# schreibfaul1/ESP32-Opus-Player

Measured on AMD Instinct MI355X. Metric: decoded 48 kHz stereo frames/sec/GPU (x real-time); HBM GB/s vs roofline, higher is better.
Workload: dtype int32 fixed-point (int16/int32 with 64-bit products); 1 GPU; celt_fb_stereo_64k; streams_per_gpu=65536

## Files before the change

__graft_entry__.py:

```python
import importlib.util
import os
import subprocess
import sys

ROOT = os.path.dirname(os.path.abspath(__file__))
PKG_DIR = os.path.join(ROOT, "esp32-opus-player_amd")
CSRC = os.path.join(PKG_DIR, "csrc")


def _load_pkg():
    name = "esp32_opus_player_amd"
    if name in sys.modules:
        return sys.modules[name]
    path = os.path.join(PKG_DIR, "__init__.py")
    spec = importlib.util.spec_from_file_location(name, path, submodule_search_locations=[PKG_DIR])
    mod = importlib.util.module_from_spec(spec)
    sys.modules[name] = mod
    spec.loader.exec_module(mod)
    return mod


def build() -> None:
    subprocess.check_call([sys.executable, os.path.join(ROOT, "tools", "gen_rom_tables.py")])
    hipcc = os.environ.get("HIPCC", "/opt/rocm/bin/hipcc")
    out = os.path.join(PKG_DIR, "libopusgpu.so")
    cmd = [hipcc, "--offload-arch=gfx950", "-O3", "-std=c++17", "-fPIC", "-shared",
           os.path.join(CSRC, "og_api.hip"), os.path.join(CSRC, "og_recon.hip"), os.path.join(CSRC, "og_parse64.hip"), os.path.join(CSRC, "og_rfc.hip"), os.path.join(CSRC, "og_silk_nb.hip"), os.path.join(CSRC, "og_silk_synth.hip"), os.path.join(CSRC, "og_compat.cpp"),
           os.path.join(CSRC, "og_pages.cpp"), os.path.join(CSRC, "og_files.cpp"),
           "-I", os.path.join(ROOT, "include"), "-pthread",
           "-o", out]
    cmd = [c for c in cmd if not c.endswith("og_compat.cpp") or os.path.exists(c)]
    flags_file = os.path.join(CSRC, "BUILD_FLAGS")
    if os.path.exists(flags_file):
        cmd += open(flags_file).read().split()
    subprocess.check_call(cmd)
    subprocess.check_call(["make", "-C", os.path.join(ROOT, "oracle"), "-s"])
    emul = os.path.join(ROOT, "tests", "emul")
    if os.path.exists(os.path.join(emul, "Makefile")):
        subprocess.check_call(["make", "-C", emul, "-s"])
    kat = os.path.join(ROOT, "tests", "gpu_kat")
    if os.path.exists(os.path.join(kat, "Makefile")):
        subprocess.check_call(["make", "-C", kat, "-s", "HIPCC=" + hipcc])
    pkg = _load_pkg()
    lib = pkg.load_lib()
    missing = [s for s in pkg.EXPORTS if not hasattr(lib, s)]
    if missing:
        raise RuntimeError(f"libopusgpu.so lacks exports: {missing}")


def smoke() -> None:
    import numpy as np
    sys.path.insert(0, os.path.join(ROOT, "tests"))
    import oracle_py
    pkg = _load_pkg()
    oracle = oracle_py.load()
    ctx = pkg.Context(0)
    n, frames = 64, 3
    for name, toc, L in (("CELT-FB", pkg.TOC_CELT_FB_STEREO, 160), ("SILK-NB", pkg.TOC_SILK_NB_STEREO, 40),
                         ("hybrid FB", pkg.TOC_HYBRID_FB_STEREO, 120)):
        pay = pkg.lcg_payloads(n, frames, L)
        ref, ok = oracle.batch_decode(2, toc, pay)
        assert ok == n * frames
        ctx.streams_alloc(n, 2)
        for f in range(frames):
            pk = [bytes([toc]) + pay[f, s].tobytes() for s in range(n)]
            pcm, res = ctx.decode_packets(np.arange(n), pk)
            assert (res == 960).all(), (name, res)
            assert (pcm == ref[:, f]).all(), f"{name}: GPU PCM differs from the oracle"
    ctx.close()
    print("smoke ok: 64 streams x 3 frames x {CELT-FB, SILK-NB, hybrid FB} bit-exact vs oracle")


if __name__ == "__main__":
    build()
    if len(sys.argv) > 1 and sys.argv[1] == "smoke":
        smoke()
```

esp32-opus-player_amd/csrc/og_api.hip:

```cpp
#include <hip/hip_runtime.h>
#include <stdio.h>
#include <stdlib.h>
#include <string.h>
#include <condition_variable>
#include <functional>
#include <memory>
#include <new>
#include <mutex>
#include <thread>
#include <vector>
#include "og_decode.hpp"
#include "og_host_framing.hpp"
#include "og_output.hpp"
#include "og_debug.hpp"

using namespace og;

static_assert(sizeof(opusgpu_frame_desc) == sizeof(FrameDesc), "descriptor layout");

#define OG_STALL_MAX_SPINS (1 << 20)
__global__ void __launch_bounds__(64) k_stream_stall(long long ticks, int max_spins) {
    const long long t0 = wall_clock64();
    for (int i = 0; i < max_spins && wall_clock64() - t0 < ticks; i++) __builtin_amdgcn_s_sleep(8);
}
// ... 212 lines not shown
            ret = BAD_ARG;
        } else if (desc_rfc(d.flags)) {
            continue;
        } else if (skip_celt && desc_mode(d.flags) == MODE_CELT) {
            continue;
        } else {
            StreamState *s = &st[d.stream];
#ifdef OG_PROF_SINGLE
            OG_PROF_INIT();
#endif
            ret = decode_frame_wave<true>(s, arena + d.offset, d.len, desc_mode(d.flags), desc_bandwidth(d.flags),
                                          desc_channels(d.flags), pcm + (size_t)f * pcm_stride, handoff ? &handoff[f] : nullptr,
                                          srecs ? &srecs[f] : nullptr, q4_only, desc_mode_after(d.flags));
#ifdef OG_PROF_SINGLE
            OG_PROF_FLUSH();
#endif
            if (ret == CONTINUE_SPLIT) continue;
        }
        if (threadIdx.x == 0) result[f] = ret;
        __syncthreads();
    }
}

extern "C" void og_launch_silk_synth(hipStream_t s, const void *descs, const void *arena, void *streams, void *pcm, void *result, int n,
                                     int n_streams, int pcm_stride, void *handoff, const void *srecs, int nb_elsewhere);
extern "C" void og_launch_silk_synth_nb(hipStream_t s, const void *descs, const void *arena, void *streams, void *pcm, void *result, int n,
                                        int n_streams, int pcm_stride, void *handoff, const void *srecs, int nb_elsewhere);

#define OG_SPARSE_WAVES 4
template <int LANES>
OG_DEV void silk_parse_kernel_body(const FrameDesc *__restrict__ descs, const u8 *__restrict__ arena, const StreamState *st, SilkRec *srecs,
                                   SilkHandoff *handoff, int n, int n_streams, SilkShadow *shadow, u32 epoch) {
    silk_tables_load();
    if ((int)threadIdx.x >= LANES) return;
    const int f = (int)blockIdx.x * LANES + (int)threadIdx.x;
    if (f >= n) return;
    const FrameDesc d = descs[f];
    const int mode = desc_mode(d.flags);
    if (d.stream < 0 || d.stream >= n_streams || mode == MODE_CELT || desc_rfc(d.flags)) return;
#ifdef OG_PROF_SPARSE
    OG_PROF_INIT();
#endif
    SilkShadow *const sh = shadow ? &shadow[d.stream] : nullptr;
    const SilkPast past(&st[d.stream], sh, epoch);
    silk_parse_lane(past, arena + d.offset, d.len, mode, desc_bandwidth(d.flags), desc_channels(d.flags), &srecs[f], &handoff[f], sh, epoch,
                    desc_mode_after(d.flags));
#ifdef OG_PROF_SPARSE
    OG_PROF_FLUSH();
#endif
}
__global__ void __launch_bounds__(64, OG_SPARSE_WAVES) k_silk_parse(const FrameDesc *__restrict__ descs, const u8 *__restrict__ arena,
                                                      const StreamState *st, SilkRec *srecs, SilkHandoff *handoff, int n,
                                                      int n_streams, SilkShadow *shadow, u32 epoch) {
    silk_parse_kernel_body<32>(descs, arena, st, srecs, handoff, n, n_streams, shadow, epoch);
}
__global__ void __launch_bounds__(64, OG_SPARSE_WAVES) k_silk_parse64(const FrameDesc *__restrict__ descs, const u8 *__restrict__ arena,
                                                        const StreamState *st, SilkRec *srecs, SilkHandoff *handoff, int n,
                                                        int n_streams, SilkShadow *shadow, u32 epoch) {
    silk_parse_kernel_body<64>(descs, arena, st, srecs, handoff, n, n_streams, shadow, epoch);
}

#define OG_SPARAMS_WAVES 4
__global__ void __launch_bounds__(64, OG_SPARAMS_WAVES) k_silk_params(const FrameDesc *__restrict__ descs, const StreamState *st, SilkRec *srecs,
                                                                       int n, int n_streams, SilkShadow *shadow, u32 epoch) {
    constexpr int FR = OG_PAR_LANES / 2;
    const int ch = (int)threadIdx.x / FR, f = (int)blockIdx.x * FR + (int)threadIdx.x % FR;
    bool act = f < n;
    FrameDesc d = {0, 0, 0, 0};
    if (act) {
        d = descs[f];
        act = !(d.stream < 0 || d.stream >= n_streams || desc_mode(d.flags) == MODE_CELT || desc_rfc(d.flags));
    }
    SilkShadow *const sh = act && shadow ? &shadow[d.stream] : nullptr;
    const SilkParPast past(act ? &st[d.stream] : st, sh, epoch);
    const int mode = desc_mode(d.flags), channels = desc_channels(d.flags);
    SilkParTask t;
    t.skip = 1;
    if (act) silk_params_channel(past, mode, desc_bandwidth(d.flags), channels, &srecs[f], ch, t);
    OG_FULL_SYNC();
    if (act) silk_params_shadow(past, t, channels, &srecs[f], ch, sh, epoch);
}

#define OG_PARSE_KERNEL_NAME k_celt_parse
#include "og_parse_kernel.hpp"
extern "C" void og_launch_celt_parse64(hipStream_t s, int grid, const void *descs, const void *arena, void *streams, void *recs, int n,
                                       int n_streams, const void *handoff, int which, int groups, unsigned *started);
extern "C" int og_celt_parse64_frames(void);

extern "C" void og_launch_celt_recon_fb(hipStream_t s, const void *descs, void *streams, const void *recs, void *rout, int n,
                                        int n_streams, int hybrid, unsigned *started, int empties);
extern "C" int og_celt_recon_fb_signals(int n);
extern "C" void og_launch_decode_rfc(hipStream_t s, const void *descs, const void *arena, void *streams, void *pcm, void *result, int n,
                                     int n_streams, int pcm_stride);
__global__ void __launch_bounds__(64, OG_RECON_WAVES) k_celt_recon(const FrameDesc *__restrict__ descs, StreamState *st,
                                                                      const ParseRec *recs, ReconOut *rout, int n,
                                                                      int n_streams, int hybrid, int rest_only) {
    unsigned long long todo = 1ull;
    int base = (int)blockIdx.x;
    if (rest_only) {
        base = (int)blockIdx.x * 64;
        const int f0 = base + (int)threadIdx.x;
        bool mine = false;
        if (f0 < n) {
            const FrameDesc d0 = descs[f0];
            const int m0 = desc_mode(d0.flags);
            if (d0.stream >= 0 && d0.stream < n_streams && (m0 == MODE_CELT || (m0 == MODE_HYBRID && hybrid)) && !desc_rfc(d0.flags)) {
                const u32 fl = recs[f0].flags;
                const bool fast = !(fl & (RF_SKIP | RF_BAD_CELT)) && ((fl >> RF_LM_SHIFT) & 3) == 3 && recs[f0].n_words < REC_MAX_WORDS &&
                                  recs[f0].n_leaves <= FAST_MAX_LEAVES;
                mine = !fast && !(m0 == MODE_HYBRID && (fl & RF_SKIP));
            }
        }
        todo = __ballot(mine);
    }
    while (todo) {
        const int f = base + (int)__builtin_ctzll(todo);
        todo &= todo - 1;
        if (f >= n) return;
        const FrameDesc d = descs[f];
        const int mode = desc_mode(d.flags);
        if (d.stream < 0 || d.stream >= n_streams || !(mode == MODE_CELT || (mode == MODE_HYBRID && hybrid)) || desc_rfc(d.flags)) continue;
        if (mode == MODE_HYBRID && (recs[f].flags & RF_SKIP)) continue;
#if !defined(OG_PROF_PARSE) && !defined(OG_PROF_SINGLE) && !defined(OG_PROF_SPARSE) && !defined(OG_PROF_SSYNTH)
        OG_PROF_INIT();
#endif
        const int pos = OG_UNI(st[d.stream].celt.ring_pos);
        const int ret = celt_recon_wave(&st[d.stream], &recs[f], mode, desc_channels(d.flags), rest_only ? RECON_REST_ONLY : RECON_ALL, desc_mode_after(d.flags));
        if (ret != RECON_NOT_MINE && threadIdx.x == 0) rout[f] = ReconOut{ret, pos};
#if !defined(OG_PROF_PARSE) && !defined(OG_PROF_SINGLE) && !defined(OG_PROF_SPARSE) && !defined(OG_PROF_SSYNTH)
        OG_PROF_FLUSH();
#endif
        __syncthreads();
    }
}

static __device__ __forceinline__ i32 pk_add_sat_i16(i32 a, i32 b) {
    typedef short s2 __attribute__((ext_vector_type(2)));
    const s2 r = __builtin_elementwise_add_sat(__builtin_bit_cast(s2, a), __builtin_bit_cast(s2, b));
    return __builtin_bit_cast(i32, r);
}
template <class T>
static __device__ __forceinline__ T *uniform_ptr(T *p) {
    const unsigned long long a = (unsigned long long)p;
    return (T *)((unsigned long long)(u32)__builtin_amdgcn_readfirstlane((int)(u32)a) |
                 (unsigned long long)(u32)__builtin_amdgcn_readfirstlane((int)(u32)(a >> 32)) << 32);
}
#define OG_POST_WAVES 5
__global__ void __launch_bounds__(64, OG_POST_WAVES) k_celt_post(const FrameDesc *__restrict__ descs, StreamState *st, const ParseRec *recs,
                                                  const ReconOut *__restrict__ rout, i32 *__restrict__ result, i16 *pcm, int n,
                                                  int n_streams, int channels, int pcm_stride, const SilkHandoff *handoff,
                                                  int modes, int others_ran) {
    constexpr int CS = 32, PCS = CS / 4, RSTEP = 64 / PCS;
    static_assert(RSTEP % 2 == 0, "a lane's rows are all of one channel");
    __shared__ __attribute__((aligned(16))) i32 tin[64][CS + 4];
    const int lane = (int)threadIdx.x;
    const int t = (int)blockIdx.x * 64 + lane;
    const int f = channels == 2 ? t >> 1 : t, c = channels == 2 ? t & 1 : 0;
    bool live = false, emit = false;
    StreamState *ss = nullptr;
    const i16 *silk = nullptr;
    int silk_n = 0;
    int pos = 0, stream = 0;
    if (f < n) {
        const FrameDesc d = descs[f];
        stream = d.stream;
        const int mode = desc_mode(d.flags);
        const bool stream_ok = d.stream >= 0 && d.stream < n_streams;
// ... 157 lines not shown
    const int per = (wide ? og_celt_parse64_frames() : OG_PL_FRAMES) * ctx->parse_groups;
    return (cnt + per - 1) / per;
}
void launch_celt_parse(opusgpu_ctx *ctx, hipStream_t q, const Step &st, size_t f0, int cnt, bool wide, bool early) {
    const StepRange r(st, f0);
    const int which = early ? (int)PARSE_CELT_ONLY : (int)PARSE_ALL, groups = early ? ctx->parse_groups : 1;
    const int per = wide ? og_celt_parse64_frames() : OG_PL_FRAMES;
    const int grid = early ? celt_parse_early_grid(ctx, cnt, wide) : (cnt + per - 1) / per;
    u32 *const started = early ? ctx->sp.d_started : nullptr;
    if (wide)
        og_launch_celt_parse64(q, grid, r.dd, st.arena, ctx->d_streams, r.recs, cnt, ctx->n_streams, r.hh, which, groups, started);
    else
        hipLaunchKernelGGL(k_celt_parse, dim3(grid), dim3(64 * OG_PL_WAVES), 0, q, r.dd, (const u8 *)st.arena, ctx->d_streams, r.recs, cnt,
                           ctx->n_streams, (const SilkHandoff *)r.hh, which, groups, started);
}
void launch_celt_recon_fb(opusgpu_ctx *ctx, hipStream_t q, const Step &st, size_t f0, int cnt, bool counts_in) {
    const StepRange r(st, f0);
    ctx->recon_fb_took_rest = counts_in && !r.hh && st.modes == 4 && og_debug().rest_in_fb;
    og_launch_celt_recon_fb(q, r.dd, ctx->d_streams, r.recs, r.rout, cnt, ctx->n_streams, r.hh ? 1 : 0, counts_in ? ctx->sp.d_started + 16 : nullptr,
                            ctx->recon_fb_took_rest ? 1 : 0);
}
void launch_celt_recon(opusgpu_ctx *ctx, hipStream_t q, const Step &st, size_t f0, int cnt) {
    if (ctx->fast_recon && ctx->recon_fb_took_rest) {
        ctx->recon_fb_took_rest = false;
        return;
    }
    const StepRange r(st, f0);
    hipLaunchKernelGGL(k_celt_recon, dim3(ctx->fast_recon ? (cnt + 63) / 64 : cnt), dim3(64), 0, q, r.dd, ctx->d_streams, (const ParseRec *)r.recs,
                       r.rout, cnt, ctx->n_streams, r.hh ? 1 : 0, ctx->fast_recon);
}
void launch_celt_post(opusgpu_ctx *ctx, hipStream_t q, const Step &st, size_t f0, int cnt, bool others) {
    const StepRange r(st, f0);
    hipLaunchKernelGGL(k_celt_post, dim3((cnt * ctx->channels + 63) / 64), dim3(64), 0, q, r.dd, ctx->d_streams, (const ParseRec *)r.recs,
                       (const ReconOut *)r.rout, r.rr, r.pp, cnt, ctx->n_streams, ctx->channels, st.pcm_stride, (const SilkHandoff *)r.hh, st.modes,
                       others ? 1 : 0);
}
void launch_silk_synth(opusgpu_ctx *ctx, hipStream_t q, const Step &st, size_t f0, int cnt, int nb_done) {
    const StepRange r(st, f0);
    og_launch_silk_synth(q, r.dd, st.arena, ctx->d_streams, r.pp, r.rr, cnt, ctx->n_streams, st.pcm_stride, r.hh, r.srecs, nb_done);
}
void launch_silk_synth_nb(opusgpu_ctx *ctx, hipStream_t q, const Step &st, size_t f0, int cnt) {
    const StepRange r(st, f0);
    og_launch_silk_synth_nb(q, r.dd, st.arena, ctx->d_streams, r.pp, r.rr, cnt, ctx->n_streams, st.pcm_stride, r.hh, r.srecs, 1);
}


extern "C" {


int opusgpu_version(void) { return 100; }

int opusgpu_ctx_create(int device, opusgpu_ctx **out) {
    if (!out || device < 0) return OPUSGPU_BAD_ARG;
    *out = nullptr;
    int count = 0;
    if (hipGetDeviceCount(&count) != hipSuccess || count <= 0 || device >= count) return OPUSGPU_ERR_NO_DEVICE;
    if (hipSetDevice(device) != hipSuccess) return OPUSGPU_ERR_NO_DEVICE;
    hipFuncAttributes attr;
    if (hipFuncGetAttributes(&attr, reinterpret_cast<const void *>(k_decode_step)) != hipSuccess) {
        (void)hipGetLastError();
        return OPUSGPU_ERR_NO_DEVICE;
    }
    opusgpu_ctx *ctx = new (std::nothrow) opusgpu_ctx();
    if (!ctx) return OPUSGPU_ALLOC_FAIL;
    ctx->device = device;
    ctx->split_celt = og_debug().split;
    ctx->split_hybrid = og_debug().split_hybrid;
    ctx->fast_recon = og_debug().fast_recon;
    ctx->parse_groups = og_debug().parse_groups;
    ctx->host_parts = og_debug().host_parts;
    if (og_debug().stall_us) {
        int khz = 0;
        if (hipDeviceGetAttribute(&khz, hipDeviceAttributeWallClockRate, device) != hipSuccess || khz <= 0) {
            (void)hipGetLastError();
            delete ctx;
            return OPUSGPU_ERR_HIP;
        }
        ctx->stall_ticks = (long long)og_debug().stall_us * khz / 1000;
    }
    if (hipStreamCreateWithFlags(&ctx->stream, hipStreamNonBlocking) != hipSuccess) {
        delete ctx;
        return OPUSGPU_ERR_HIP;
    }
    *out = ctx;
    return OPUSGPU_OK;
}

void opusgpu_ctx_destroy(opusgpu_ctx *ctx) {
    if (!ctx) return;
    (void)hipSetDevice(ctx->device);
    (void)hipStreamSynchronize(ctx->stream);
    (void)hipFree(ctx->d_streams);
    (void)hipFree(ctx->d_descs);
    (void)hipFree(ctx->d_arena);
    (void)hipFree(ctx->d_pcm);
    (void)hipFree(ctx->d_result);
    pipeline_destroy(ctx);
    for (int i = 0; i < 6; i++) {
        (void)hipFree(ctx->d_recs[i]);
        (void)hipFree(ctx->d_rout[i]);
    }
    for (int i = 0; i < OG_SILK_SETS; i++) {
        (void)hipFree(ctx->d_handoff[i]);
        (void)hipFree(ctx->d_srecs[i]);
    }
    (void)hipFree(ctx->d_shadow);
    (void)hipHostFree(ctx->h_pcm);
    (void)hipHostFree(ctx->h_res);
    (void)hipHostFree(ctx->h_arena);
    (void)hipHostFree(ctx->h_descs);
    (void)hipFree(ctx->d_crc_tables);
    for (hipEvent_t e : ctx->ev_piece)
        if (e) (void)hipEventDestroy(e);
    for (hipEvent_t e : ctx->ev_part)
        if (e) (void)hipEventDestroy(e);
    if (ctx->copy_stream) (void)hipStreamDestroy(ctx->copy_stream);
    (void)hipStreamDestroy(ctx->stream);
    delete ctx;
}

const char *opusgpu_last_error(const opusgpu_ctx *ctx) { return ctx ? ctx->err : "no context"; }
int opusgpu_set_mode(opusgpu_ctx *ctx, int mode) {
    if (!ctx || (mode != OPUSGPU_MODE_REFERENCE && mode != OPUSGPU_MODE_RFC)) return OPUSGPU_BAD_ARG;
    ctx->mode = mode;
    return OPUSGPU_OK;
}
int opusgpu_get_mode(const opusgpu_ctx *ctx) { return ctx ? ctx->mode : OPUSGPU_MODE_REFERENCE; }
int opusgpu_set_pipeline(opusgpu_ctx *ctx, int on) {
    if (!ctx) return OPUSGPU_BAD_ARG;
    HIPCHK(ctx, hipSetDevice(ctx->device));
    if (on)
        if (int rc = pipeline_create(ctx)) return rc;
    if ((on != 0) != (ctx->pipeline != 0)) {
        HIPCHK(ctx, hipDeviceSynchronize());
        ctx->sp.drained();
        ctx->sp.last_kind = 0;
        ctx->sp.shadow_epoch++;
    }
    ctx->pipeline = on ? 1 : 0;
    return OPUSGPU_OK;
}
int opusgpu_get_pipeline(const opusgpu_ctx *ctx) { return ctx ? ctx->pipeline : 0; }
size_t opusgpu_stream_state_bytes(void) { return sizeof(StreamState); }
int opusgpu_stream_count(const opusgpu_ctx *ctx) { return ctx ? ctx->n_streams : 0; }
int opusgpu_stream_channels(const opusgpu_ctx *ctx) { return ctx ? ctx->channels : 0; }

int opusgpu_streams_reset(opusgpu_ctx *ctx, int first, int count, int full) {
    if (!ctx || first < 0 || count < 0 || first + count > ctx->n_streams) return OPUSGPU_BAD_ARG;
    if (count == 0) return OPUSGPU_OK;
    HIPCHK(ctx, hipSetDevice(ctx->device));
    if (int rc = sync_in_flight(ctx)) return rc;
    ctx->sp.drained();
    ctx->sp.shadow_epoch++;
    hipLaunchKernelGGL(k_stream_init, dim3(count), dim3(64), 0, ctx->stream, ctx->d_streams, first, count, ctx->channels,
                       full ? 1 : 0);
    HIPCHK(ctx, hipGetLastError());
    HIPCHK(ctx, hipStreamSynchronize(ctx->stream));
    for (int i = first; i < first + count; i++) ctx->last_count[i] = ctx->last_flags[i] = 0;
    return OPUSGPU_OK;
}

int opusgpu_streams_alloc(opusgpu_ctx *ctx, int n_streams, int channels) {
    if (!ctx || n_streams <= 0 || (channels != 1 && channels != 2)) return OPUSGPU_BAD_ARG;
    HIPCHK(ctx, hipSetDevice(ctx->device));
    HIPCHK(ctx, hipStreamSynchronize(ctx->stream));
    if (int rc = sync_in_flight(ctx)) return rc;
// ... 385 lines not shown
```

esp32-opus-player_amd/csrc/og_celt_parse.hpp:

```cpp
#pragma once
#include "og_celt.hpp"
#include "og_celt_rec.hpp"

namespace og {

#ifndef OG_PL_LANES
#define OG_PL_LANES (OG_NLANES >= 32 ? 32 : OG_NLANES)
#endif
#ifndef OG_PL_WAVES
#define OG_PL_WAVES 1
#endif
#ifdef OG_HOST_EMUL
#define OG_PWAVE 0
#define OG_PCOL OG_LANE
#else
#define OG_PWAVE ((int)(threadIdx.x >> 6))
#define OG_PCOL ((int)(threadIdx.x & 63))
#endif
#define OG_PL_FRAMES (OG_PL_LANES * OG_PL_WAVES)
struct ParseLds {
    i8 fine_quant[NBANDS][OG_PL_LANES];
    i8 tf_prio[NBANDS][OG_PL_LANES];
    union {
        i16 bandE[2 * NBANDS][OG_PL_LANES];
        struct {
            u32 bw[NBANDS][OG_PL_LANES];
        } al;
        i32 stack[4][5][OG_PL_LANES];
    } u;
};
#ifdef OG_PARSE_DYN_LDS
extern __shared__ __attribute__((aligned(16))) unsigned char og_dyn_lds[];
#define PLs (reinterpret_cast<ParseLds *>(og_dyn_lds))
#else
OG_LDS ParseLds PLs[OG_PL_WAVES];
#endif
#define PL PLs[OG_PWAVE]

struct ParseTabLds {
    i16 eband[NBANDS + 1], logn[NBANDS];
    u16 pulse_idx[105];
    u32 pulse_v[392];
    u8 pulse_bits[392], band_alloc[231], pulse_caps[168], log2_frac[24], eprob[336];
};
#ifdef OG_PARSE_DYN_LDS
#define PT (*reinterpret_cast<ParseTabLds *>(og_dyn_lds + sizeof(ParseLds) * OG_PL_WAVES))
#define OG_PARSE_LDS_BYTES (sizeof(ParseLds) * OG_PL_WAVES + sizeof(ParseTabLds))
#else
OG_LDS ParseTabLds PT;
#define OG_PARSE_LDS_BYTES 0
#endif
struct RomLds {
    static OG_MEMBER i32 eband(int i) { return PT.eband[i]; }
    static OG_MEMBER i32 logn(int i) { return PT.logn[i]; }
    static OG_MEMBER i32 pulse_idx(int i) { return PT.pulse_idx[i]; }
    static OG_MEMBER i32 pulse_bits(int i) { return PT.pulse_bits[i]; }
    static OG_MEMBER i32 band_alloc(int i) { return PT.band_alloc[i]; }
    static OG_MEMBER i32 pulse_caps(int i) { return PT.pulse_caps[i]; }
    static OG_MEMBER i32 log2_frac(int i) { return PT.log2_frac[i]; }
    static OG_MEMBER i32 eprob(int i) { return PT.eprob[i]; }
};
OG_DEV void parse_tables_load() {
    OG_FOR_LANES(i, NBANDS + 1) PT.eband[i] = rom_eband[i];
    OG_FOR_LANES(i, NBANDS) PT.logn[i] = rom_logn[i];
    OG_FOR_LANES(i, 105) PT.pulse_idx[i] = rom_pulse_idx[i];
    OG_FOR_LANES(i, 392) PT.pulse_bits[i] = rom_pulse_bits[i];
    OG_FOR_LANES(i, 392) PT.pulse_v[i] = rom_pulse_v[i];
    OG_FOR_LANES(i, 231) PT.band_alloc[i] = rom_band_alloc[i];
    OG_FOR_LANES(i, 168) PT.pulse_caps[i] = rom_pulse_caps[i];
    OG_FOR_LANES(i, 24) PT.log2_frac[i] = rom_log2_frac[i];
    OG_FOR_LANES(i, 336) PT.eprob[i] = rom_eprob[i];
    OG_FULL_SYNC();
}

struct TfResView {
    i8 *p;
    OG_MEMBER operator int() const { return (int)(i8)((u8)*p << 4) >> 4; }
    OG_MEMBER void operator=(int v) const { *p = (i8)((*p & 0xF0) | (v & 15)); }
};
struct FinePrioView {
    i8 *p;
    OG_MEMBER operator int() const { return (*p >> 4) & 1; }
    OG_MEMBER void operator=(int v) const { *p = (i8)((*p & ~0x10) | ((v & 1) << 4)); }
};
struct LaneArr {
// ... 10 lines not shown
        for (int i = 0; i < NBANDS; i++) w[i] = *reinterpret_cast<const u32 *>(&rest[2 * i]);
        for (int i = 0; i < NBANDS; i++) {
            PL.u.bandE[2 * i][OG_PCOL] = (i16)(w[i] & 0xffff);
            PL.u.bandE[2 * i + 1][OG_PCOL] = (i16)(w[i] >> 16);
        }
    }
    typedef u16 __attribute__((may_alias)) u16a;
    typedef i32 __attribute__((may_alias)) i32a;
    OG_MEMBER i32 &pulses(int i) const { return pl[i]; }
    OG_MEMBER i32a &alloc_bits(int i) const { return *reinterpret_cast<i32a *>(&PL.u.al.bw[i][OG_PCOL]); }
    OG_MEMBER void pulses_rest(int start, int end) const {
        i32 v[24];
        for (int i = 0; i < 24; i++) v[i] = (i >= start && i < end) ? (i32)PL.u.al.bw[i < NBANDS ? i : 0][OG_PCOL] : 0;
#ifdef OG_HOST_EMUL
        for (int i = 0; i < NBANDS; i++) pl[i] = v[i];
#else
        typedef i32 i32x4 __attribute__((ext_vector_type(4)));
        for (int i = 0; i < 24; i += 4) *reinterpret_cast<i32x4 *>(&pl[i]) = i32x4{v[i], v[i + 1], v[i + 2], v[i + 3]};
#endif
        for (int i = 0; i < NBANDS; i++) pk[i] = (i16)v[i];
    }
    OG_MEMBER i8 &fine_quant(int i) const { return PL.fine_quant[i][OG_PCOL]; }
    OG_MEMBER FinePrioView fine_prio(int i) const { return FinePrioView{&PL.tf_prio[i][OG_PCOL]}; }
    OG_MEMBER TfResView tf_res(int i) const { return TfResView{&PL.tf_prio[i][OG_PCOL]}; }
    OG_MEMBER void boost_put(int i, int n, int) const {
#ifdef OG_HOST_EMUL
        if (n < 0 || n > 127) __builtin_trap();
#endif
        PL.fine_quant[i][OG_PCOL] = (i8)n;
    }
    OG_MEMBER i32 boost(int i, int C, int LM) const { return (i32)PL.fine_quant[i][OG_PCOL] * dynalloc_quanta<RomLds>(i, LM, C); }
    OG_MEMBER u16a &bits1(int i) const { return reinterpret_cast<u16a *>(&PL.u.al.bw[i][OG_PCOL])[0]; }
    OG_MEMBER u16a &bits2(int i) const { return reinterpret_cast<u16a *>(&PL.u.al.bw[i][OG_PCOL])[1]; }
    OG_MEMBER i16 &bandE(int i) const { return PL.u.bandE[i][OG_PCOL]; }
};

struct RecWriter {
    ParseRec *rec;
    int nw, nl, ncoef = 0;
    int job = 0;
    OG_MEMBER void word(u32 w) {
        if (nw < REC_MAX_WORDS) rec->words[nw] = w;
        nw++;
    }
    OG_MEMBER int reserve() { return nw++; }
    OG_MEMBER void patch(int at, u32 w) {
        if (at < REC_MAX_WORDS) rec->words[at] = w;
    }
    OG_MEMBER void leaf(int x, int N, int K, int B, i32 gain, int off, u32 idx) {
        if (nl < REC_MAX_LEAVES) {
            const u32 geom = (u32)x | (u32)N << 11 | (u32)K << 19 | (u32)(B - 1) << 27;
            const u32 aux = (u32)(gain & 0xffff) | (u32)off << 16 | (u32)job << 20;
#ifdef OG_HOST_EMUL
            rec->leaf[nl].idx = idx; rec->leaf[nl].geom = geom; rec->leaf[nl].aux = aux; rec->leaf[nl].pad = 0;
#else
            typedef u32 u32x4 __attribute__((ext_vector_type(4)));
            *reinterpret_cast<u32x4 *>(&rec->leaf[nl]) = u32x4{idx, geom, aux, 0u};
#endif
        }
        nl++;
        ncoef += N;
    }
    OG_MEMBER int band_begin() { return nw = (nw + 3) & ~3; }
    OG_MEMBER void words4(u32 w0, u32 w1, u32 w2, u32 w3) {
        if (nw + 4 <= REC_MAX_WORDS) {
#ifdef OG_HOST_EMUL
            rec->words[nw] = w0; rec->words[nw + 1] = w1; rec->words[nw + 2] = w2; rec->words[nw + 3] = w3;
#else
            typedef u32 u32x4 __attribute__((ext_vector_type(4)));
            *reinterpret_cast<u32x4 *>(&rec->words[nw]) = u32x4{w0, w1, w2, w3};
#endif
        }
        nw += 4;
    }
};

OG_DEV u32 isqrt24(u32 val) {
    u32 g = (u32)__builtin_sqrtf((float)val);
    g -= g * g > val;
    g += (g + 1) * (g + 1) <= val;
    return g;
}

OG_DEV void split_theta_lane(RcLane &rc, int band, Split &sc, int N, i32 &b, int B0, int LM) {
    int itheta = 0;
    const int pulse_cap = RomLds::logn(band) + LM * (1 << BITRES);
    const int offset = (pulse_cap >> 1) - 4;
    const int qn = compute_qn(N, b, offset, pulse_cap, 0);
    const u32 tell = rc_tell_frac(rc);
    if (qn != 1) {
        const bool uni = B0 > 1;
        const int h = qn >> 1;
        const int ftb = uni ? OG_MAX(ilog((u32)qn) - 8, 0) : 0;
        const u32 ft = uni ? (u32)(qn >> ftb) + 1 : (u32)((h + 1) * (h + 1));
        const u32 fm = rc_decode(rc, ft);
        const bool low = fm < (u32)(h * (h + 1) >> 1);
        const u32 root = isqrt24(8 * (low ? fm : ft - fm - 1) + 1);
        const int it = low ? (int)((root - 1) >> 1) : (int)((2u * (u32)(qn + 1) - root) >> 1);
        const int fs_t = low ? it + 1 : qn + 1 - it;
        const u32 fl_t = low ? (u32)(it * (it + 1) >> 1) : ft - (u32)(fs_t * (fs_t + 1) >> 1);
        const u32 fl = uni ? fm : fl_t, fs = uni ? 1u : (u32)fs_t;
        rc_update(rc, fl, fl + fs, ft);
        itheta = uni ? (int)fm : it;
        if (ftb) {
            const u32 t = fm << ftb | rc_bits(rc, (unsigned)ftb);
            if (t > (u32)qn) rc.error = 1;
            itheta = (int)OG_MIN(t, (u32)qn);
        }
        itheta = (int)udiv((u32)(itheta * 16384), (u32)qn);
    }
    const int qalloc = (int)(rc_tell_frac(rc) - tell);
    b -= qalloc;
    int imid, iside, delta;
    if (itheta == 0) {
        imid = 32767;
        iside = 0;
        delta = -16384;
    } else if (itheta == 16384) {
        imid = 0;
        iside = 32767;
        delta = 16384;
    } else {
        imid = bitexact_cos(itheta);
        iside = bitexact_cos(16384 - itheta);
        delta = frac_mul16((N - 1) << 7, bitexact_log2tan(iside, imid));
    }
    sc.inv = 0;
    sc.imid = imid;
    sc.iside = iside;
    sc.delta = delta;
    sc.itheta = itheta;
    sc.qalloc = qalloc;
}

OG_DEV int parse_tree(RcLane &rc, RecWriter &out, int band, i32 &remaining_bits, int x, int N, i32 b, int B, int LM, i32 gain,
                      int has_low, int silent) {
    int depth = 0, off = 0, n_fill = 0;
    const int jpos = out.reserve(), first_pvq = out.nl;
    for (;;) {
        OG_MARK(41);
        for (;;) {
            if (!(LM != -1 && b > pulse_cache_max<RomLds>(band, LM) + 12 && N > 2)) break;
            const int B0 = B;
            Split sc;
            N >>= 1;
            LM -= 1;
            B = (B + 1) >> 1;
            split_theta_lane(rc, band, sc, N, b, B0, LM);
            i32 delta = sc.delta;
            const int itheta = sc.itheta;
            if (B0 > 1 && (itheta & 0x3fff)) {
                if (itheta > 8192)
                    delta -= delta >> (4 - LM);
                else
                    delta = OG_MIN(0, delta + (N << BITRES >> (5 - LM)));
            }
            const i32 mbits = OG_MAX(0, OG_MIN(b, (b - delta) / 2));
            const i32 sbits = b - mbits;
            remaining_bits -= sc.qalloc;
            const int mid_first = mbits >= sbits;
            const int off_side = off + (B0 >> 1), silent_mid = silent | (itheta == 16384), silent_side = silent | (itheta == 0);
            const i32 gain_mid = tr16(mul16_p15(gain, sc.imid)), gain_side = tr16(mul16_p15(gain, sc.iside));
#ifdef OG_HOST_EMUL
            if (x + N >= 2048 || N > 255 || LM + 1 > 7 || B > 31 || off_side > 15) __builtin_trap();
#endif
            i32 *F = &PL.u.stack[depth][0][OG_PCOL];
            F[0 * OG_PL_LANES] = (i32)((u32)(mid_first ? x + N : x) | (u32)N << 11 | (u32)(LM + 1) << 19 | (u32)B << 22 |
                                       (u32)(mid_first ? off_side : off) << 27 | (u32)(mid_first ? silent_side : silent_mid) << 31);
            F[1 * OG_PL_LANES] = mid_first ? mbits : sbits;
            F[2 * OG_PL_LANES] = mid_first ? sbits : mbits;
            F[3 * OG_PL_LANES] = remaining_bits;
            F[4 * OG_PL_LANES] = ((mid_first ? gain_side : gain_mid) & 0xffff) | (itheta != (mid_first ? 0 : 16384)) << 16;
            depth++;
            if (mid_first) {
                b = mbits;
                gain = gain_mid;
                silent = silent_mid;
            } else {
                x += N;
                b = sbits;
                gain = gain_side;
                off = off_side;
                silent = silent_side;
            }
        }
        {
            OG_MARK(42);
            int q = bits2pulses<RomLds>(band, LM, b), curr_bits = pulses2bits<RomLds>(band, LM, q);
            remaining_bits -= curr_bits;
            while (remaining_bits < 0 && q > 0) {
                remaining_bits += curr_bits;
                q--;
                curr_bits = pulses2bits<RomLds>(band, LM, q);
                remaining_bits -= curr_bits;
            }
            const int K = q ? get_pulses(q) : 0;
            OG_MARK(43);
            if (K)
                out.leaf(x, N, K, B, gain, off, rc_uint(rc, PT.pulse_v[pulse_cache<RomLds>(band, LM) + q]));
            else if (!silent) {
                out.word((u32)off << LW_OFF_SHIFT | (u32)(B - 1) << LW_B_SHIFT | (u32)N << LW_N_SHIFT);
                out.word((u32)x | (u32)(gain & 0xffff) << 11);
                n_fill++;
            }
        }
        OG_MARK(44);
        if (depth == 0) break;
        {
            depth--;
// ... 256 lines not shown
```

esp32-opus-player_amd/csrc/og_parse64.hip:

```cpp
#include <hip/hip_runtime.h>
#define OG_PL_LANES 64
#define OG_PL_WAVES 2
#define OG_PARSE_KERNEL_NAME k_celt_parse64
#define OG_PARSE_DYN_LDS 1
#define OG_PARSE_WAVES_PER_SIMD 3
#ifndef OG_PARSE_NUM_VGPR
#define OG_PARSE_NUM_VGPR 152
#endif
#include "og_parse_kernel.hpp"

extern "C" void og_launch_celt_parse64(hipStream_t s, int grid, const void *descs, const void *arena, void *streams, void *recs, int n,
                                       int n_streams, const void *handoff, int which, int groups, unsigned *started) {
    hipLaunchKernelGGL(k_celt_parse64, dim3(grid), dim3(64 * OG_PL_WAVES), OG_PARSE_LDS_BYTES, s, (const FrameDesc *)descs, (const u8 *)arena, (StreamState *)streams,
                       (ParseRec *)recs, n, n_streams, (const SilkHandoff *)handoff, which, groups, started);
}
extern "C" int og_celt_parse64_frames(void) { return OG_PL_FRAMES; }

static_assert(sizeof(ParseLds) == (size_t)OG_PL_LANES * (2 * NBANDS + 4 * NBANDS), "a parse wave's LDS: fine_quant, tf_prio and one word per band");
static_assert(sizeof(ParseLds) <= 8064 && OG_PARSE_LDS_BYTES + 256 <= 16 * 1280, "k_celt_parse64's workgroup no longer fits 16 LDS granules");
static_assert((128 - 2 * ((OG_PARSE_LDS_BYTES + 256 + 1279) / 1280)) / 5 >= 19, "fewer than 19 reconstruction workgroups per CU beside two parse workgroups");
extern "C" int og_celt_parse64_lds_bytes(void) { return (int)OG_PARSE_LDS_BYTES; }
```

esp32-opus-player_amd/csrc/og_parse_kernel.hpp:

```cpp
#pragma once
#include "og_celt_parse.hpp"

using namespace og;

enum { PARSE_ALL = 0, PARSE_CELT_ONLY = 1, PARSE_HYBRID_ONLY = 2 };
#ifndef OG_PARSE_WAVES_PER_SIMD
#define OG_PARSE_WAVES_PER_SIMD 2
#endif
#ifdef OG_PARSE_NUM_VGPR
#define OG_PARSE_VGPR_ATTR __attribute__((amdgpu_num_vgpr(OG_PARSE_NUM_VGPR / 2)))
#else
#define OG_PARSE_VGPR_ATTR
#endif
__global__ void OG_PARSE_VGPR_ATTR __attribute__((amdgpu_waves_per_eu(OG_PARSE_WAVES_PER_SIMD, 8))) __launch_bounds__(64 * OG_PL_WAVES) OG_PARSE_KERNEL_NAME(const FrameDesc *__restrict__ descs, const u8 *__restrict__ arena,
                                                      StreamState *st, ParseRec *recs, int n, int n_streams,
                                                      const SilkHandoff *handoff, int which, int groups, u32 *started) {
    if (started && threadIdx.x == 0) __hip_atomic_fetch_add(started, 1u, __ATOMIC_RELAXED, __HIP_MEMORY_SCOPE_SYSTEM);
    const bool lane_on = (int)(threadIdx.x & 63) < OG_PL_LANES;
    const int f0 = (int)blockIdx.x * groups * OG_PL_FRAMES + OG_PWAVE * OG_PL_LANES + OG_PCOL;
    if (which != PARSE_ALL) {
        bool mine = false;
        for (int g = 0; g < groups; g++) {
            const int f = f0 + g * OG_PL_FRAMES;
            if (lane_on && f < n) {
                const int m0 = desc_mode(descs[f].flags);
                mine |= which == PARSE_CELT_ONLY ? m0 == MODE_CELT : m0 == MODE_HYBRID;
            }
        }
        if (!__syncthreads_or(mine)) return;
    }
    parse_tables_load();
    if (!lane_on) return;
    for (int g = 0; g < groups; g++) {
        const int f = f0 + g * OG_PL_FRAMES;
        if (f >= n) break;
        const FrameDesc d = descs[f];
        const int mode = desc_mode(d.flags);
        if (d.stream < 0 || d.stream >= n_streams || !(mode == MODE_CELT || (mode == MODE_HYBRID && handoff)) || desc_rfc(d.flags)) continue;
        if ((which == PARSE_CELT_ONLY && mode != MODE_CELT) || (which == PARSE_HYBRID_ONLY && mode != MODE_HYBRID)) continue;
#ifdef OG_PROF_PARSE
        OG_PROF_INIT();
#endif
        celt_parse_lane(&st[d.stream], arena + d.offset, d.len, desc_channels(d.flags), &recs[f], mode == MODE_HYBRID ? &handoff[f] : nullptr);
#ifdef OG_PROF_PARSE
        OG_PROF_FLUSH();
#endif
    }
}
```

esp32-opus-player_amd/csrc/og_range.hpp:

```cpp
#pragma once
#include "og_state.hpp"

namespace og {

OG_LDS FrameLds S;

struct Rc {
    u32 storage, end_offs, end_window;
    i32 nend_bits, nbits_total;
    u32 offs, rng, val, ext;
    i32 rem, error;
};
typedef u32 og_u32x4 __attribute__((ext_vector_type(4)));
struct RcLane : Rc {
    const u8 *buf;
#ifndef OG_HOST_EMUL
    const __attribute__((address_space(1))) og_u32x4 *chunks;
    const __attribute__((address_space(1))) u32 *words;
    u32 fshift, shift;
    i32 last_chunk, last_word;
    og_u32x4 f_cur, f_next;
    u32 b_cur, b_next;
    i32 f_idx, b_idx;
#endif
};

OG_DEV int rc_next_byte(Rc &rc) { return rc.offs < rc.storage ? S.pkt[rc.offs++] : 0; }
OG_DEV int rc_next_byte_end(Rc &rc) {
    return rc.end_offs < rc.storage ? S.pkt[rc.storage - ++rc.end_offs] : 0;
}
#ifdef OG_HOST_EMUL
OG_DEV void rc_lane_attach(RcLane &rc, const u8 *buf, u32 len) {
    rc.buf = buf;
    (void)len;
}
OG_DEV void rc_lane_resume(RcLane &rc) {}
OG_DEV int rc_next_byte(RcLane &rc) { return rc.offs < rc.storage ? rc.buf[rc.offs++] : 0; }
OG_DEV int rc_next_byte_end(RcLane &rc) { return rc.end_offs < rc.storage ? rc.buf[rc.storage - ++rc.end_offs] : 0; }
#else
OG_DEV u32 rc_lane_word(const RcLane &rc, i32 w) { return (w >= 0 && w <= rc.last_word) ? rc.words[w] : 0u; }
OG_DEV og_u32x4 rc_lane_chunk(const RcLane &rc, i32 w) { return (w >= 0 && w <= rc.last_chunk) ? rc.chunks[w] : og_u32x4{0u, 0u, 0u, 0u}; }
OG_DEV void rc_lane_attach(RcLane &rc, const u8 *buf, u32 len) {
    rc.buf = buf;
    const unsigned long long a = (unsigned long long)buf;
    rc.chunks = (const __attribute__((address_space(1))) og_u32x4 *)(a & ~15ull);
    rc.words = (const __attribute__((address_space(1))) u32 *)(a & ~3ull);
    rc.fshift = (u32)(a & 15ull);
    rc.shift = (u32)(a & 3ull);
    rc.last_chunk = len ? (i32)((rc.fshift + len - 1) >> 4) : -1;
    rc.last_word = len ? (i32)((rc.shift + len - 1) >> 2) : -1;
    rc.f_idx = 0;
    rc.f_cur = rc_lane_chunk(rc, 0);
    rc.f_next = rc_lane_chunk(rc, 1);
    rc.b_idx = rc.last_word;
    rc.b_cur = rc_lane_word(rc, rc.b_idx);
    rc.b_next = rc_lane_word(rc, rc.b_idx - 1);
}
OG_DEV void rc_lane_resume(RcLane &rc) {
    rc.f_idx = (i32)((rc.offs + rc.fshift) >> 4);
    rc.f_cur = rc_lane_chunk(rc, rc.f_idx);
    rc.f_next = rc_lane_chunk(rc, rc.f_idx + 1);
    rc.b_idx = rc.end_offs < rc.storage ? (i32)((rc.storage - rc.end_offs - 1 + rc.shift) >> 2) : rc.last_word;
    rc.b_cur = rc_lane_word(rc, rc.b_idx);
    rc.b_next = rc_lane_word(rc, rc.b_idx - 1);
}
OG_DEV int rc_next_byte(RcLane &rc) {
    if (rc.offs >= rc.storage) return 0;
    const u32 pos = rc.offs++ + rc.fshift;
    const i32 w = (i32)(pos >> 4);
    if (w != rc.f_idx) {
        rc.f_cur = rc.f_next;
        rc.f_idx = w;
        rc.f_next = rc_lane_chunk(rc, w + 1);
    }
    const bool up = (pos & 8u) != 0;
    const u32 lo = up ? rc.f_cur.z : rc.f_cur.x, hi = up ? rc.f_cur.w : rc.f_cur.y;
    return (int)__builtin_amdgcn_perm(hi, lo, 0x0c0c0c00u | (pos & 7u));
}
OG_DEV int rc_next_byte_end(RcLane &rc) {
    if (rc.end_offs >= rc.storage) return 0;
    const u32 pos = rc.storage - ++rc.end_offs + rc.shift;
    const i32 w = (i32)(pos >> 2);
    if (w != rc.b_idx) {
        rc.b_cur = rc.b_next;
        rc.b_idx = w;
        rc.b_next = rc_lane_word(rc, w - 1);
    }
    return (int)((rc.b_cur >> (8 * (pos & 3))) & 255u);
}
#endif

template <class R>
OG_DEV void rc_renorm(R &rc) {
    while (rc.rng <= (1u << 23)) {
        rc.nbits_total += 8;
        rc.rng <<= 8;
        int sym = rc.rem;
        rc.rem = rc_next_byte(rc);
        sym = (sym << 8 | rc.rem) >> 1;
        rc.val = ((rc.val << 8) + (255u & ~(u32)sym)) & 0x7FFFFFFFu;
    }
}

template <class R>
OG_DEV void rc_init(R &rc, u32 len) {
    rc.storage = len;
    rc.end_offs = 0;
    rc.end_window = 0;
    rc.nend_bits = 0;
    rc.nbits_total = 9;
    rc.offs = 0;
    rc.rng = 128;
    rc.rem = rc_next_byte(rc);
    rc.val = rc.rng - 1 - (rc.rem >> 1);
    rc.ext = 0;
    rc.error = 0;
    rc_renorm(rc);
}

template <class R>
OG_DEV i32 rc_tell(const R &rc) { return rc.nbits_total - ilog(rc.rng); }

template <class R>
OG_DEV u32 rc_tell_frac(const R &rc) {
    u32 nbits = (u32)rc.nbits_total << 3;
    int l = ilog(rc.rng);
    u32 r = rc.rng >> (l - 16);
    u32 b = (r >> 12) - 8;
    u32 corr = b == 0 ? 35733u : b == 1 ? 38967u : b == 2 ? 42495u : b == 3 ? 46340u
             : b == 4 ? 50535u : b == 5 ? 55109u : b == 6 ? 60097u : 65535u;
    b += r > corr;
    return nbits - (u32)((l << 3) + b);
}

template <class R>
OG_DEV u32 rc_decode(R &rc, u32 ft) {
    rc.ext = rc.rng / ft;
    u32 s = rc.val / rc.ext;
    return ft - OG_MIN(s + 1, ft);
}

template <class R>
OG_DEV u32 rc_decode_bin(R &rc, unsigned bits) {
    rc.ext = rc.rng >> bits;
    u32 s = rc.val / rc.ext, top = 1u << bits;
    return top - OG_MIN(s + 1u, top);
}

template <class R>
OG_DEV void rc_update(R &rc, u32 fl, u32 fh, u32 ft) {
    u32 s = rc.ext * (ft - fh);
    rc.val -= s;
    rc.rng = fl > 0 ? rc.ext * (fh - fl) : rc.rng - s;
    rc_renorm(rc);
}

template <class R>
OG_DEV int rc_bit_logp(R &rc, unsigned logp) {
    u32 r = rc.rng, d = rc.val, s = r >> logp;
    int ret = d < s;
    if (!ret) rc.val = d - s;
    rc.rng = ret ? s : r - s;
    rc_renorm(rc);
    return ret;
}

template <class R>
OG_DEV int rc_icdf(R &rc, const u8 *icdf, unsigned ftb) {
    u32 s = rc.rng, d = rc.val, r = s >> ftb, t;
    int ret = -1;
    do {
        t = s;
        s = r * icdf[++ret];
    } while (d < s);
    rc.val = d - s;
    rc.rng = t - s;
    rc_renorm(rc);
    return ret;
}

#ifndef OG_HOST_EMUL
OG_DEV int rc_icdf(Rc &rc, const u8 *icdf, unsigned ftb) {
    const u32 d = rc.val, r = rc.rng >> ftb;
    const u32 s_l = r * (u32)icdf[OG_LANE];
    const u64 hit = __ballot(d >= s_l);
    const int ret = (int)__builtin_ctzll(hit);
    const u32 s = (u32)__builtin_amdgcn_readlane((int)s_l, ret);
    const u32 t = ret ? (u32)__builtin_amdgcn_readlane((int)s_l, ret - 1) : rc.rng;
    rc.val = d - s;
    rc.rng = t - s;
    rc_renorm(rc);
    return ret;
}
#endif

template <class R>
OG_DEV u32 rc_bits(R &rc, unsigned bits) {
    u32 window = rc.end_window;
    int available = rc.nend_bits;
    if ((u32)available < bits) {
        do {
            window |= (u32)rc_next_byte_end(rc) << available;
            available += 8;
        } while (available <= 24);
    }
    u32 ret = window & ((1u << bits) - 1u);
    rc.end_window = window >> bits;
    rc.nend_bits = available - (int)bits;
    rc.nbits_total += bits;
    return ret;
}

template <class R>
OG_DEV u32 rc_uint(R &rc, u32 ft_in) {
    ft_in--;
    int ftb = ilog(ft_in);
    if (ftb > 8) {
        ftb -= 8;
        u32 ft = (ft_in >> ftb) + 1;
        u32 s = rc_decode(rc, ft);
        rc_update(rc, s, s + 1, ft);
        u32 t = s << ftb | rc_bits(rc, ftb);
        if (t <= ft_in) return t;
        rc.error = 1;
        return ft_in;
    }
    ft_in++;
    u32 s = rc_decode(rc, ft_in);
    rc_update(rc, s, s + 1, ft_in);
    return s;
// ... 46 lines not shown
```

Before: 52.35 million frames/s.

## Tabulate split-theta trig values and use reciprocal-based division in range decoder

Replaces the per-band bitexact_cos/log2tan and division computations in split_theta_lane with a lookup into a device-global table holding packed itheta/imid/iside/log2tan entries for every even qn up to 256. The table is filled by a one-time kernel at context creation. It also replaces the integer divisions in the RcLane range decoder's rc_decode and rc_decode_bin with float-reciprocal estimates plus correction steps. The aim is to cut ALU-heavy integer division and trig work in the parse kernel, at the cost of extra global-memory gathers and reliance on bounded operand ranges for exactness.

```diff
diff --git a/__graft_entry__.py b/__graft_entry__.py
--- a/__graft_entry__.py
+++ b/__graft_entry__.py
@@ -41,6 +41,9 @@
     kat = os.path.join(ROOT, "tests", "gpu_kat")
     if os.path.exists(os.path.join(kat, "Makefile")):
         subprocess.check_call(["make", "-C", kat, "-s", "HIPCC=" + hipcc])
+    forms = os.path.join(ROOT, "tests", "parse_forms")
+    if os.path.exists(os.path.join(forms, "Makefile")):
+        subprocess.check_call(["make", "-C", forms, "-s", "HIPCC=" + hipcc])
     pkg = _load_pkg()
     lib = pkg.load_lib()
     missing = [s for s in pkg.EXPORTS if not hasattr(lib, s)]
diff --git a/esp32-opus-player_amd/csrc/og_api.hip b/esp32-opus-player_amd/csrc/og_api.hip
--- a/esp32-opus-player_amd/csrc/og_api.hip
+++ b/esp32-opus-player_amd/csrc/og_api.hip
@@ -318,7 +318,21 @@
 }
 
 #define OG_PARSE_KERNEL_NAME k_celt_parse
+#define OG_PARSE_TABLES_KERNEL_NAME k_celt_parse_tables
 #include "og_parse_kernel.hpp"
+extern "C" void og_launch_celt_parse64_tables(hipStream_t s);
+static bool parse_tables_fill(int device, hipStream_t q) {
+    static std::mutex mu;
+    static std::vector<bool> filled;
+    std::lock_guard<std::mutex> lock(mu);
+    if ((size_t)device < filled.size() && filled[(size_t)device]) return true;
+    hipLaunchKernelGGL(k_celt_parse_tables, dim3(1), dim3(256), 0, q);
+    og_launch_celt_parse64_tables(q);
+    if (hipGetLastError() != hipSuccess || hipStreamSynchronize(q) != hipSuccess) return false;
+    if (filled.size() <= (size_t)device) filled.resize((size_t)device + 1, false);
+    filled[(size_t)device] = true;
+    return true;
+}
 extern "C" void og_launch_celt_parse64(hipStream_t s, int grid, const void *descs, const void *arena, void *streams, void *recs, int n,
                                        int n_streams, const void *handoff, int which, int groups, unsigned *started);
 extern "C" int og_celt_parse64_frames(void);
@@ -642,6 +656,12 @@
         delete ctx;
         return OPUSGPU_ERR_HIP;
     }
+    if (!parse_tables_fill(device, ctx->stream)) {
+        (void)hipGetLastError();
+        (void)hipStreamDestroy(ctx->stream);
+        delete ctx;
+        return OPUSGPU_ERR_HIP;
+    }
     *out = ctx;
     return OPUSGPU_OK;
 }
diff --git a/esp32-opus-player_amd/csrc/og_celt_parse.hpp b/esp32-opus-player_amd/csrc/og_celt_parse.hpp
--- a/esp32-opus-player_amd/csrc/og_celt_parse.hpp
+++ b/esp32-opus-player_amd/csrc/og_celt_parse.hpp
@@ -1,6 +1,7 @@
 #pragma once
 #include "og_celt.hpp"
 #include "og_celt_rec.hpp"
+#include "og_theta_table.hpp"
 
 namespace og {
 
@@ -177,12 +178,21 @@
     return g;
 }
 
+#if defined(OG_HOST_EMUL) && !defined(OG_THETA_ARITH)
+#define OG_THETA_ARITH 1
+#endif
+#ifndef OG_THETA_TAP
+#define OG_THETA_TAP(qn, itheta) ((void)0)
+#endif
 OG_DEV void split_theta_lane(RcLane &rc, int band, Split &sc, int N, i32 &b, int B0, int LM) {
     int itheta = 0;
     const int pulse_cap = RomLds::logn(band) + LM * (1 << BITRES);
     const int offset = (pulse_cap >> 1) - 4;
     const int qn = compute_qn(N, b, offset, pulse_cap, 0);
     const u32 tell = rc_tell_frac(rc);
+#ifndef OG_THETA_ARITH
+    ThetaEntry te = theta_entry_zero();
+#endif
     if (qn != 1) {
         const bool uni = B0 > 1;
         const int h = qn >> 1;
@@ -202,11 +212,21 @@
             if (t > (u32)qn) rc.error = 1;
             itheta = (int)OG_MIN(t, (u32)qn);
         }
+#ifdef OG_THETA_ARITH
         itheta = (int)udiv((u32)(itheta * 16384), (u32)qn);
+#else
+        te = theta_tab_at(qn, itheta);
+#endif
     }
     const int qalloc = (int)(rc_tell_frac(rc) - tell);
     b -= qalloc;
     int imid, iside, delta;
+#ifndef OG_THETA_ARITH
+    itheta = theta_itheta(te);
+    imid = theta_imid(te);
+    iside = theta_iside(te);
+    delta = theta_delta(te, N);
+#else
     if (itheta == 0) {
         imid = 32767;
         iside = 0;
@@ -220,6 +240,8 @@
         iside = bitexact_cos(16384 - itheta);
         delta = frac_mul16((N - 1) << 7, bitexact_log2tan(iside, imid));
     }
+#endif
+    OG_THETA_TAP(qn, itheta);
     sc.inv = 0;
     sc.imid = imid;
     sc.iside = iside;
diff --git a/esp32-opus-player_amd/csrc/og_div_forms.hpp b/esp32-opus-player_amd/csrc/og_div_forms.hpp
--- /dev/null
+++ b/esp32-opus-player_amd/csrc/og_div_forms.hpp
@@ -0,0 +1,29 @@
+#pragma once
+#include <stdint.h>
+
+#if defined(__HIPCC__) && !defined(OG_HOST_EMUL)
+#define OG_DIVF static __host__ __device__ __forceinline__
+#else
+#define OG_DIVF static inline
+#endif
+
+namespace og {
+
+OG_DIVF float div_rcp_below(float rcp_d) { return __builtin_bit_cast(float, __builtin_bit_cast(uint32_t, rcp_d) - 8u); }
+
+OG_DIVF uint32_t div_small_quotient(uint32_t n, uint32_t d, float rcp_d) {
+    const uint32_t e = (uint32_t)((float)n * div_rcp_below(rcp_d));
+    const uint32_t rem = n - e * d;
+    return e + (rem >= d);
+}
+
+OG_DIVF uint32_t div_small_divisor(uint32_t n, uint32_t d, float rcp_d) {
+    const float r = div_rcp_below(rcp_d);
+    const uint32_t e1 = (uint32_t)((float)n * r);
+    const uint32_t rem1 = n - e1 * d;
+    const uint32_t e2 = (uint32_t)((float)rem1 * r);
+    const uint32_t rem2 = rem1 - (e2 & 0xffffffu) * (d & 0xffffffu);
+    return e1 + e2 + (rem2 >= d);
+}
+
+}
diff --git a/esp32-opus-player_amd/csrc/og_parse64.hip b/esp32-opus-player_amd/csrc/og_parse64.hip
--- a/esp32-opus-player_amd/csrc/og_parse64.hip
+++ b/esp32-opus-player_amd/csrc/og_parse64.hip
@@ -2,6 +2,7 @@
 #define OG_PL_LANES 64
 #define OG_PL_WAVES 2
 #define OG_PARSE_KERNEL_NAME k_celt_parse64
+#define OG_PARSE_TABLES_KERNEL_NAME k_celt_parse64_tables
 #define OG_PARSE_DYN_LDS 1
 #define OG_PARSE_WAVES_PER_SIMD 3
 #ifndef OG_PARSE_NUM_VGPR
@@ -15,6 +16,7 @@
                        (ParseRec *)recs, n, n_streams, (const SilkHandoff *)handoff, which, groups, started);
 }
 extern "C" int og_celt_parse64_frames(void) { return OG_PL_FRAMES; }
+extern "C" void og_launch_celt_parse64_tables(hipStream_t s) { hipLaunchKernelGGL(k_celt_parse64_tables, dim3(1), dim3(256), 0, s); }
 
 static_assert(sizeof(ParseLds) == (size_t)OG_PL_LANES * (2 * NBANDS + 4 * NBANDS), "a parse wave's LDS: fine_quant, tf_prio and one word per band");
 static_assert(sizeof(ParseLds) <= 8064 && OG_PARSE_LDS_BYTES + 256 <= 16 * 1280, "k_celt_parse64's workgroup no longer fits 16 LDS granules");
diff --git a/esp32-opus-player_amd/csrc/og_parse_kernel.hpp b/esp32-opus-player_amd/csrc/og_parse_kernel.hpp
--- a/esp32-opus-player_amd/csrc/og_parse_kernel.hpp
+++ b/esp32-opus-player_amd/csrc/og_parse_kernel.hpp
@@ -47,3 +47,5 @@
 #endif
     }
 }
+
+__global__ void __launch_bounds__(256) OG_PARSE_TABLES_KERNEL_NAME() { theta_tab_fill(g_theta_tab, (int)threadIdx.x, (int)blockDim.x); }
diff --git a/esp32-opus-player_amd/csrc/og_range.hpp b/esp32-opus-player_amd/csrc/og_range.hpp
--- a/esp32-opus-player_amd/csrc/og_range.hpp
+++ b/esp32-opus-player_amd/csrc/og_range.hpp
@@ -1,5 +1,8 @@
 #pragma once
 #include "og_state.hpp"
+#ifndef OG_HOST_EMUL
+#include "og_div_forms.hpp"
+#endif
 
 namespace og {
 
@@ -146,6 +149,21 @@
     u32 s = rc.val / rc.ext, top = 1u << bits;
     return top - OG_MIN(s + 1u, top);
 }
+
+#if !defined(OG_HOST_EMUL) && !defined(OG_RC_GENERIC_DIV)
+OG_DEV float rc_rcp(u32 d) { return __builtin_amdgcn_rcpf((float)d); }
+static_assert(((128 + 1) * (128 + 1)) <= (1 << 16) && (1 << 16) + (1 << 9) < (1 << 17), "rc_decode(RcLane): ft, val / ext");
+OG_DEV u32 rc_decode(RcLane &rc, u32 ft) {
+    rc.ext = div_small_divisor(rc.rng, ft, rc_rcp(ft));
+    const u32 s = div_small_quotient(rc.val, rc.ext, rc_rcp(rc.ext));
+    return ft - OG_MIN(s + 1, ft);
+}
+OG_DEV u32 rc_decode_bin(RcLane &rc, unsigned bits) {
+    rc.ext = rc.rng >> bits;
+    const u32 s = div_small_quotient(rc.val, rc.ext, rc_rcp(rc.ext)), top = 1u << bits;
+    return top - OG_MIN(s + 1u, top);
+}
+#endif
 
 template <class R>
 OG_DEV void rc_update(R &rc, u32 fl, u32 fh, u32 ft) {
diff --git a/esp32-opus-player_amd/csrc/og_theta_table.hpp b/esp32-opus-player_amd/csrc/og_theta_table.hpp
--- /dev/null
+++ b/esp32-opus-player_amd/csrc/og_theta_table.hpp
@@ -0,0 +1,52 @@
+#pragma once
+#include "og_celt_math.hpp"
+
+namespace og {
+
+constexpr int THETA_QN_MAX = 256;
+constexpr int THETA_TAB_ENTRIES = (THETA_QN_MAX / 2 + 1) * (THETA_QN_MAX / 2 + 1) - 1;
+static_assert(THETA_TAB_ENTRIES == 16640, "one row of qn + 1 angles per even qn in 2..256");
+
+OG_DEV int theta_tab_row(int qn) { return (qn >> 1) * (qn >> 1) - 1; }
+static_assert(THETA_QN_MAX / 2 * (THETA_QN_MAX / 2) - 1 + THETA_QN_MAX == THETA_TAB_ENTRIES - 1, "the last row ends the table");
+
+struct ThetaEntry { u32 lo, hi; };
+OG_DEV ThetaEntry theta_entry(int qn, int j) {
+    const int itheta = (int)udiv((u32)(j * 16384), (u32)qn);
+    int imid = 32767, iside = 0, lt = 0;
+    if (itheta == 16384) {
+        imid = 0;
+        iside = 32767;
+    } else if (itheta != 0) {
+        imid = bitexact_cos(itheta);
+        iside = bitexact_cos(16384 - itheta);
+        lt = bitexact_log2tan(iside, imid);
+    }
+    return ThetaEntry{(u32)itheta | (u32)imid << 16, (u32)iside | (u32)(u16)lt << 16};
+}
+OG_DEV int theta_itheta(ThetaEntry e) { return (int)(e.lo & 0xffffu); }
+OG_DEV int theta_imid(ThetaEntry e) { return (int)(e.lo >> 16); }
+OG_DEV int theta_iside(ThetaEntry e) { return (int)(e.hi & 0xffffu); }
+OG_DEV i32 theta_delta(ThetaEntry e, int N) {
+    const int itheta = theta_itheta(e);
+    const i32 d = frac_mul16((N - 1) << 7, (i32)e.hi >> 16);
+    return itheta == 0 ? -16384 : itheta == 16384 ? 16384 : d;
+}
+OG_DEV ThetaEntry theta_entry_zero() { return ThetaEntry{32767u << 16, 0u}; }
+
+OG_DEV void theta_tab_fill(ThetaEntry *tab, int tid, int nthreads) {
+    for (int qn = 2; qn <= THETA_QN_MAX; qn += 2)
+        for (int j = tid; j <= qn; j += nthreads) tab[theta_tab_row(qn) + j] = theta_entry(qn, j);
+}
+
+#ifndef OG_HOST_EMUL
+static __device__ __attribute__((aligned(8))) ThetaEntry g_theta_tab[THETA_TAB_ENTRIES];
+OG_DEV ThetaEntry theta_tab_at(int qn, int j) {
+    const u32 at = OG_MIN((u32)(theta_tab_row(qn) + j), (u32)(THETA_TAB_ENTRIES - 1));
+    typedef u32 u32x2 __attribute__((ext_vector_type(2)));
+    const u32x2 v = ((const __attribute__((address_space(1))) u32x2 *)g_theta_tab)[at];
+    return ThetaEntry{v.x, v.y};
+}
+#endif
+
+}
```

After: 52.78 million frames/s, median of 6. Within noise of the previous version (+0.8%).
